# andres2631996/bikg_graph_explainability_public

Hardware: AMD Instinct MI355X
Metric: perturbation-samples/sec (masked GNN fwd) per query node; 1/2/4/8 GPU (higher is better)
Workload: dtype fp32

## Files before the change

bikg_graph_explainability_public_amd/_lib.py:

```python
import ctypes
import os

import torch

_HERE = os.path.dirname(os.path.abspath(__file__))
LIB_PATH = os.path.join(_HERE, "libxpgnn.so")
ABI_VERSION = 27
MAX_TERMS = 8

ACT = {None: 0, "identity": 0, "relu": 1, "sigmoid": 2, "tanh": 3, "leaky_relu": 4, "elu": 5}
TERM = {"gcn": 0, "mean": 1, "root": 2, "att": 3, "sum": 4, "max": 5, "rel": 6}
REL_NORM = {"mean": 0, "sum": 1}
POOL = {None: 0, "mean": 1, "sum": 2, "max": 3}

c_i32, c_i64, c_f32, c_vp = ctypes.c_int32, ctypes.c_int64, ctypes.c_float, ctypes.c_void_p


class NativeLibraryError(RuntimeError):
    pass


class FitExchangeError(RuntimeError):
    """The multi-workgroup surrogate fit's cross-workgroup exchange timed out (its workgroups
    were not all resident on the GPU at once): the fit's outputs are invalid."""
# ... 32 lines not shown


class WlmParams(ctypes.Structure):
    _fields_ = [("lr", c_f32), ("l1_lambda", c_f32), ("beta1", c_f32), ("beta2", c_f32),
                ("eps", c_f32), ("weight_decay", c_f32)]


_SIGS = {
    "xpg_abi_version": ([], c_i32),
    "xpg_last_error": ([], ctypes.c_char_p),
    "xpg_pack_masks": ([c_vp, c_i64, c_i64, c_vp, c_vp], c_i32),
    "xpg_unpack_masks": ([c_vp, c_i64, c_i64, c_vp, c_vp], c_i32),
    "xpg_sample_shapley": ([ctypes.c_uint64, c_i64, c_i64, c_i64, c_vp, c_vp], c_i32),
    "xpg_sample_shapley_counts": ([ctypes.c_uint64, c_i64, c_i64, c_i64, c_vp, c_vp, c_vp], c_i32),
    "xpg_sample_shapley_dev": ([c_vp, c_i64, c_i64, c_i64, c_vp, c_vp], c_i32),
    "xpg_sample_shapley_sets": ([c_vp, c_i32, c_i64, c_i64, c_vp, c_vp], c_i32),
    "xpg_plan_arrays_build": ([c_i64, c_i32, c_vp, c_vp, c_vp, c_vp, c_vp, c_i64, c_i32, c_vp, c_vp], c_i32),
    "xpg_plan_arrays_take": ([c_vp, c_vp], c_i32),
    "xpg_plan_arrays_free": ([c_vp], c_i32),
    "xpg_mt19937_mask_bits": ([c_vp, c_vp, c_vp, c_i64, c_i64, c_vp], c_i32),
    "xpg_mt19937_repeat_draws": ([c_vp, c_vp, c_vp, c_i32, c_i64, ctypes.c_float, ctypes.c_float, c_i32, c_vp,
                                  c_vp], c_i32),
    "xpg_mt19937_community_bits": ([c_vp, c_vp, c_vp, c_i64, c_i32, c_vp, c_vp, c_vp, c_i32, c_i64,
                                    c_vp], c_i32),
    "xpg_sample_communities": ([ctypes.c_uint64, c_i64, c_i64, c_i32, c_vp, c_i32, c_i64, c_i32, c_vp, c_vp,
                                c_vp, c_vp, c_vp], c_i32),
    "xpg_sample_communities_rows": ([ctypes.c_uint64, c_i64, c_i64, c_i64, c_i32, c_vp, c_i32, c_i64, c_i32, c_vp, c_vp,
                                c_vp, c_vp, c_vp], c_i32),
    "xpg_sampler_describe": ([c_i32, c_i64, c_i64, c_i32, c_i32, ctypes.c_char_p, ctypes.c_size_t], c_i32),
    "xpg_edge_keep": ([c_vp, c_i64, c_i64, c_vp, c_vp, c_i64, c_vp, c_vp], c_i32),
    "xpg_rows_no_edge": ([c_vp, c_i64, c_i64, c_vp, c_vp, c_i64, c_vp, c_vp], c_i32),
    "xpg_popcount_rows": ([c_vp, c_i64, c_i64, c_vp, c_vp], c_i32),
    "xpg_shap_kernel": ([c_vp, c_i64, c_i64, c_vp, c_vp], c_i32),
    "xpg_dense": ([c_vp, c_i64, c_i64, c_vp, c_i64, c_i64, c_vp, c_i64, c_i64, ctypes.c_int,
                   c_vp, c_i64, c_vp], c_i32),
    "xpg_forward_workspace": ([ctypes.POINTER(ForwardPlanDesc), c_i64,
                               ctypes.POINTER(ctypes.c_size_t)], c_i32),
    "xpg_masked_forward": ([ctypes.POINTER(ForwardPlanDesc), c_vp, c_i64, c_vp, c_vp,
                            ctypes.c_size_t, c_vp], c_i32),
    "xpg_forward_describe": ([ctypes.POINTER(ForwardPlanDesc), c_i64, ctypes.c_char_p,
                              ctypes.c_size_t], c_i32),
    "xpg_wide_variants": ([ctypes.c_char_p, ctypes.c_size_t], c_i32),
    "xpg_pool_workspace": ([c_i64, c_i64, c_i64, ctypes.POINTER(ctypes.c_size_t)], c_i32),
    "xpg_pool_rows": ([c_vp, c_i64, c_i64, c_i64, c_i32, c_vp, c_vp, ctypes.c_size_t, c_vp], c_i32),
    "xpg_pool_describe": ([c_i64, c_i64, c_i64, c_i32, ctypes.c_char_p, ctypes.c_size_t], c_i32),
    "xpg_profile_enable": ([ctypes.c_int], c_i32),
    "xpg_profile_read": ([c_vp, c_vp, c_i32], c_i32),
    "xpg_wlm_workspace": ([c_i64, c_i64, c_i64, c_i64, ctypes.POINTER(ctypes.c_size_t)], c_i32),
    "xpg_wlm_plan": ([c_i64, c_i64, c_i64, c_i64, ctypes.POINTER(c_i32), ctypes.POINTER(c_i32)], c_i32),
    "xpg_wlm_fit": ([c_i64, c_vp, c_i64, c_i64, c_i64, c_vp, c_vp, ctypes.POINTER(WlmParams), c_i64,
                     c_vp, c_vp, c_vp, c_vp, c_vp, c_vp, c_vp, ctypes.c_size_t, c_vp], c_i32),
    "xpg_wlm_fit_from": ([c_i64, c_vp, c_i64, c_i64, c_i64, c_vp, c_vp, ctypes.POINTER(WlmParams), c_vp,
                          c_vp, c_vp, c_vp, c_vp, c_vp, c_vp, c_vp, ctypes.c_size_t, c_vp], c_i32),
    "xpg_wlm_prepare": ([c_i64, c_vp, c_i64, c_i64, c_i64, c_vp, c_vp, ctypes.POINTER(WlmParams), c_vp,
                         c_vp, c_vp, c_vp, c_vp, ctypes.c_size_t, c_vp], c_i32),
    "xpg_wlm_fit_prepared": ([c_i64, c_vp, c_i64, c_i64, c_i64, c_vp, ctypes.POINTER(WlmParams), c_vp,
                              c_vp, c_vp, c_vp, c_vp, c_vp, c_vp, ctypes.c_size_t, c_vp], c_i32),
    "xpg_wlm_fit_steps": ([c_i64, c_vp, c_i64, c_i64, c_i64, c_vp, ctypes.POINTER(WlmParams), c_vp, c_vp,
                           c_vp, c_vp, ctypes.c_size_t, c_vp], c_i32),
    "xpg_wlm_fit_losses": ([c_i64, c_i64, c_i64, c_i64, c_vp, ctypes.POINTER(WlmParams), c_vp, c_vp, c_vp,
                            c_vp, ctypes.c_size_t, c_vp], c_i32),
    "xpg_khop_workspace": ([c_i64, c_i64, ctypes.POINTER(ctypes.c_size_t)], c_i32),
    "xpg_khop_subgraph": ([c_vp, c_i64, c_i64, c_i64, c_i32, c_vp, c_vp, c_vp, c_vp, c_vp, c_vp,
                           ctypes.c_size_t, c_vp], c_i32),
}

# ... 62 lines not shown
```

bikg_graph_explainability_public_amd/csrc/xpgnn.hip:

```cpp
#include <hip/hip_runtime.h>

#include <algorithm>
#include <cmath>
#include <cstdlib>
#include <cstdint>
#include <cstring>
#include <string>
#include <mutex>
#include <unordered_map>
#include <unordered_set>
#include <vector>

#include "../../include/xpgnn.h"
#include "host_rng.h"
#include "plan_host.h"

namespace {

thread_local std::string g_err;

int fail(int code, const std::string& msg) {
  g_err = msg;
  return code;
}
// ... 456 lines not shown
  if (k < 0.0 || k > n) return 0.0;
  double kx = k;
  if (kx > n / 2 && n > 0) kx = n - kx;
  if (kx >= 0 && kx < 20) {
    double num = 1.0, den = 1.0;
    const int kk = static_cast<int>(kx);
    for (int i = 1; i < 1 + kk; ++i) {
      num *= i + n - kx;
      den *= i;
      if (fabs(num) > 1e50) {
        num /= den;
        den = 1.0;
      }
    }
    return num / den;
  }
  return exp(lgamma(n + 1.0) - lgamma(k + 1.0) - lgamma(n - k + 1.0));
}

__device__ __forceinline__ double clean_inf(double v) { return (isinf(v) || isnan(v)) ? 0.0 : v; }

__device__ double block_sum_d(double v, double* red) {
#pragma unroll
  for (int off = 32; off > 0; off >>= 1) v += __shfl_xor(v, off, 64);
  const int wv = threadIdx.x >> 6, nw = blockDim.x >> 6;
  __syncthreads();
  if ((threadIdx.x & 63) == 0) red[wv] = v;
  __syncthreads();
  double s = 0.0;
  for (int i = 0; i < nw; ++i) s += red[i];
  return s;
}

__global__ void k_shap_exact(const int32_t* __restrict__ cnt, int64_t rows, int64_t cols,
                             double* __restrict__ out) {
  const int64_t r = blockIdx.x * (int64_t)blockDim.x + threadIdx.x;
  if (r >= rows) return;
  const int64_t Mi = cols - 1;
  const double M = static_cast<double>(Mi);
  const int64_t k = cnt[r];
  const double choose = binom_d(M + 1.0, static_cast<double>(k));
  out[r] = clean_inf(M / (choose * static_cast<double>(Mi + 1 - k) * static_cast<double>(k)));
}

__device__ __forceinline__ double shap_approx_row(int64_t k, int64_t Mi, int ref) {
  const double M = static_cast<double>(Mi);
  int64_t idx = static_cast<int64_t>(static_cast<float>(k * 1000) / static_cast<float>(Mi));
  idx = idx < 0 ? 0 : (idx > ref - 1 ? ref - 1 : idx);
  const double choose = (binom_d(static_cast<double>(ref), static_cast<double>(idx)) + 1e-10) * M / 1000.0;
  return M / (choose * static_cast<double>(k) * static_cast<double>(Mi - k));
}

__global__ void k_shap_approx_rows(const int32_t* __restrict__ cnt, int64_t rows, int64_t cols,
                                   double* __restrict__ out) {
  const int64_t r = blockIdx.x * (int64_t)blockDim.x + threadIdx.x;
  if (r < rows) out[r] = shap_approx_row(cnt[r], cols - 1, 1000);
}

__global__ __launch_bounds__(1024) void k_shap_approx_finish(const int32_t* __restrict__ cnt,
                                                             int64_t rows, int64_t cols,
                                                             double* __restrict__ out) {
  const int64_t Mi = cols - 1;
  int ref = 1000;
  for (;;) {
    bool found = false;
    for (int64_t base = 0; base < rows && !found; base += blockDim.x) {
      const int64_t r = base + threadIdx.x;
      found = __syncthreads_or(r < rows && !(out[r] == 0.0)) != 0;
    }
    if (found) break;
    ref = static_cast<int>(0.9 * static_cast<double>(ref));
    if (!(ref > 0)) break;
    __syncthreads();
    for (int64_t r = threadIdx.x; r < rows; r += blockDim.x) out[r] = shap_approx_row(cnt[r], Mi, ref);
    __syncthreads();
  }
}

__global__ void k_shap_clean(int64_t rows, double* __restrict__ out) {
  const int64_t r = blockIdx.x * (int64_t)blockDim.x + threadIdx.x;
  if (r < rows) out[r] = clean_inf(out[r]);
}

__device__ __forceinline__ float half_wave_sum(float x) {
  x += __int_as_float(__builtin_amdgcn_update_dpp(0, __float_as_int(x), 0xB1, 0xF, 0xF, false));
  x += __int_as_float(__builtin_amdgcn_update_dpp(0, __float_as_int(x), 0x4E, 0xF, 0xF, false));
  x += __int_as_float(__builtin_amdgcn_update_dpp(0, __float_as_int(x), 0x124, 0xF, 0xF, false));
  x += __int_as_float(__builtin_amdgcn_update_dpp(0, __float_as_int(x), 0x128, 0xF, 0xF, false));
  const auto r = __builtin_amdgcn_permlane16_swap(__float_as_uint(x), __float_as_uint(x), false, false);
  return __uint_as_float(r[0]) + __uint_as_float(r[1]);
}

template <int NT, bool HEAD = false>
__global__ __launch_bounds__(256) void k_dense(const float* __restrict__ A, int64_t M, int64_t lda,
                                               const float* __restrict__ W, int64_t ldw, int k_pad,
                                               const float* __restrict__ bias, int n_real, int act,
                                               float* __restrict__ C, int64_t ldc,
                                               const int32_t* __restrict__ row_type, int64_t type_mod,
                                               int bias_ld, int n_groups, const float* __restrict__ hw = nullptr,
                                               const float* __restrict__ hb = nullptr, int hact = 0,
                                               float* __restrict__ y = nullptr) {
  const int lane = threadIdx.x & 63;
  const int64_t wv = blockIdx.x * (int64_t)(blockDim.x >> 6) + (threadIdx.x >> 6);
  const int cg = static_cast<int>(wv % n_groups);
  const int64_t m0 = (wv / n_groups) * 32;
  if (m0 >= M) return;
  const int c0 = cg * NT * 32;
  W += (int64_t)c0 * ldw;
  bias += c0;
  C += c0;
  if (HEAD) hw += c0;
  n_real -= c0;
  const int i = lane & 31, h = lane >> 5;
  const int64_t arow = m0 + i;
// ... 1156 lines not shown
    }
  }
}

__device__ __forceinline__ void rows_dense(const float* A, int K, const float* W, int ldw,
                                           const float* __restrict__ bias, int n_real, int n_pad, int act,
                                           float* out, int wave, int lane) {
  for (int o0 = wave * 4; o0 < n_pad; o0 += 4 * kRowsWaves) {
    float acc[4] = {0.f, 0.f, 0.f, 0.f};
#pragma unroll 2
    for (int kc = 0; kc < K; kc += 4) {
      float av[4];
      float4 wv[4];
#pragma unroll
      for (int i = 0; i < 4; ++i) av[i] = A[(kc + i) * 64 + lane];
#pragma unroll
      for (int q = 0; q < 4; ++q) wv[q] = *reinterpret_cast<const float4*>(W + (int64_t)(o0 + q) * ldw + kc);
#pragma unroll
      for (int q = 0; q < 4; ++q) {
        acc[q] = fmaf(av[0], wv[q].x, acc[q]);
        acc[q] = fmaf(av[1], wv[q].y, acc[q]);
        acc[q] = fmaf(av[2], wv[q].z, acc[q]);
        acc[q] = fmaf(av[3], wv[q].w, acc[q]);
      }
    }
#pragma unroll
    for (int q = 0; q < 4; ++q) {
      const int o = o0 + q;
      if (o < n_pad) out[o * 64 + lane] = o < n_real ? act_apply(acc[q] + bias[o], act) : 0.f;
    }
  }
}

template <int FS, bool SUMK>
__device__ __forceinline__ void rows_h1(const RowsFwdArgs& a, const float* lds, int s, int fo, int lane,
                                        float (&h)[FS]) {
  const int* li = reinterpret_cast<const int*>(lds);
#pragma unroll
  for (int f = 0; f < FS; ++f) h[f] = 0.f;
  const int tf0 = li[a.o_l1tgt + s];
  for (int k = 0; k < a.n_terms1; ++k) {
    const int kind = a.kind1[k], r = a.rel1[k];
    const float* T = lds + a.o_tab + k * a.n0 * a.f1_pad + fo;
    const float* dvr = lds + a.o_dv + r * a.n0 * 64 + lane;
    float cself, cedge_t;
    if (kind == XPG_TERM_ROOT) {
      cself = 1.f;
      cedge_t = 0.f;
    } else {
      const float kt = lds[a.o_kt + (r * a.n1 + tf0) * 64 + lane];
      if (kind == XPG_TERM_GCN) {
        const float dt = inv_sqrt_deg(kt);
        cself = dt * dt;
        cedge_t = kt >= 0.f ? dt : 0.f;
      } else {
        const int sm = li[a.o_l1smul + r * a.n1 + s];
        const float cnt = kt + static_cast<float>(sm);
        const float inv = SUMK && kind == XPG_TERM_SUM ? 1.f : 1.f / (cnt > 1.f ? cnt : 1.f);
        cself = kt >= 0.f ? static_cast<float>(sm) * inv : 0.f;
        cedge_t = kt >= 0.f ? inv : 0.f;
      }
    }
    {
      float v[FS];
      ld_fs<FS>(T + tf0 * a.f1_pad, v);
#pragma unroll
      for (int f = 0; f < FS; ++f) h[f] = fmaf(cself, v[f], h[f]);
    }
    if (kind == XPG_TERM_ROOT) continue;
    const int* pp = li + a.o_l1ptr + r * (a.n1 + 1);
    const int e0 = pp[s], e1 = pp[s + 1];
    const float gmul = kind == XPG_TERM_GCN ? cedge_t : 0.f;
    const float mmul = kind == XPG_TERM_GCN ? 0.f : cedge_t;
    constexpr int EB = 4;
    for (int wb = e0; wb < e1; wb += 64) {
      const int ne = min(64, e1 - wb);
      const int vsrc = li[a.o_l1f0 + wb + min(lane, ne - 1)];
      for (int i0 = 0; i0 < ne; i0 += EB) {
        int u[EB];
        float d[EB], v[EB][FS];
#pragma unroll
        for (int q = 0; q < EB; ++q) u[q] = rdl(vsrc, min(i0 + q, ne - 1));
#pragma unroll
        for (int q = 0; q < EB; ++q) d[q] = dvr[u[q] * 64];
#pragma unroll
        for (int q = 0; q < EB; ++q) ld_fs<FS>(T + u[q] * a.f1_pad, v[q]);
#pragma unroll
        for (int q = 0; q < EB; ++q) {
          const float valid = static_cast<float>(i0 + q < ne);
          const float c = valid * fmaf(d[q], gmul, fminf(d[q] * 1e30f, 1.f) * mmul);
#pragma unroll
          for (int f = 0; f < FS; ++f) h[f] = fmaf(c, v[q][f], h[f]);
        }
      }
    }
  }
#pragma unroll
  for (int f = 0; f < FS; ++f) {
    const int fg = fo + f;
    h[f] = fg < a.f1_out ? act_apply(h[f] + a.bias1[fg], a.act1) : 0.f;
  }
}

template <int FS, bool SUMK = false>
__global__ __launch_bounds__(1024) void k_rows_forward(const RowsFwdArgs a) {
  extern __shared__ __attribute__((aligned(16))) float lds[];
  int* li = reinterpret_cast<int*>(lds);
  const int tid = threadIdx.x, lane = tid & 63;
  const int wave = __builtin_amdgcn_readfirstlane(tid >> 6);
  __shared__ int blk_s;
  if (a.ctl) {
    if (tid == 0) {
      const int x = xcc_id();
      const int busy = __hip_atomic_load(g_xcd_busy + x, __ATOMIC_RELAXED, __HIP_MEMORY_SCOPE_AGENT);
      const int cap = a.cus_per_xcd - busy > 1 ? a.cus_per_xcd - busy : 1;
      const int slot = __hip_atomic_fetch_add(a.ctl + 1 + x, 1, __ATOMIC_RELAXED, __HIP_MEMORY_SCOPE_AGENT);
      blk_s = slot < cap ? 0 : -1;
    }
    __syncthreads();
    if (blk_s < 0) return;
  }
#ifdef XPG_WLM_STAMPS
  uint64_t stamp_acc[8] = {0, 0, 0, 0, 0, 0, 0, 0};
  uint64_t stamp_last = __builtin_amdgcn_s_memtime();
#endif
  {
    const int n4 = a.n0 * a.f1_pad / 4;
    for (int k = 0; k < a.n_terms1; ++k) {
// ... 2301 lines not shown
  for (int i = 0; i < kStepDw; ++i) d[i] = __builtin_amdgcn_readlane(v, i);
  WlmStep s;
  s.ybar = __hiloint2double(static_cast<int>(d[1]), static_cast<int>(d[0]));
  s.ksum = __hiloint2double(static_cast<int>(d[3]), static_cast<int>(d[2]));
  s.vy = __hiloint2double(static_cast<int>(d[5]), static_cast<int>(d[4]));
  s.cg = __hiloint2double(static_cast<int>(d[7]), static_cast<int>(d[6]));
  s.step_size = __uint_as_float(d[8]);
  s.bc2_sqrt = __uint_as_float(d[9]);
  s.inv_bc2 = __uint_as_float(d[10]);
  s.pad = 0.f;
  return s;
}

template <int B>
__device__ __forceinline__ float quad_bcast(float x) {
  return __int_as_float(__builtin_amdgcn_mov_dpp(__float_as_int(x), B | (B << 2) | (B << 4) | (B << 6), 0xF, 0xF, false));
}

__device__ __forceinline__ void quad_table_entries(float x, float* dst) {
  const float x0 = quad_bcast<0>(x), x1 = quad_bcast<1>(x), x2 = quad_bcast<2>(x), x3 = quad_bcast<3>(x);
  const int q = threadIdx.x & 3;
#pragma unroll
  for (int i = 0; i < 4; ++i) {
    const int vv = 4 * q + i;
    float s = 0.f;
    s += (vv & 1) ? x0 : 0.f;
    s += (vv & 2) ? x1 : 0.f;
    s += (vv & 4) ? x2 : 0.f;
    s += (vv & 8) ? x3 : 0.f;
    dst[vv] = s;
  }
}

template <int CPL, int STG>
__global__ __launch_bounds__(1024) void k_wlm_fit_mc(
    const uint32_t* __restrict__ bits, const uint32_t* __restrict__ colbits, int64_t rows, int cols, int words,
    int batch, int bw, int P, int wpp, int n_ds, int64_t n_fits, int xcd_local,
    const double* __restrict__ kern,
    const WlmStep* __restrict__ stp, xpg_wlm_params Pm, float* __restrict__ wg, float* __restrict__ mg,
    float* __restrict__ vg, float* __restrict__ p_hist, float* __restrict__ w_hist, uint64_t* xp,
    uint32_t* err, uint32_t spin_limit, int fault_part, uint32_t epoch_host, int plain_ok,
    const uint32_t* __restrict__ ep_dev) {
  uint32_t epoch = (epoch_host + (ep_dev ? *ep_dev : 0u)) & 0xFFFFu;
  if (epoch == 0u) epoch = 1u;
  static_assert(sizeof(WlmStep) == 48, "WlmStep is read as 12 dwords");
  extern __shared__ __attribute__((aligned(16))) char smem[];
  __shared__ int abort_s;
  const int tid = threadIdx.x, lane = tid & 63, wave = tid >> 6;
  if (tid == 0) abort_s = 0;
  int64_t f;
  int part;
  if (xcd_local) {
    const int64_t k = blockIdx.x >> 3, g = k / P;
    part = static_cast<int>(k - g * P);
    f = g * 8 + (blockIdx.x & 7);
    if (f >= n_fits) return;
  } else {
    f = blockIdx.x / P;
    part = static_cast<int>(blockIdx.x - f * P);
  }
  const int my_xcc = xcc_id();
  if (tid == 0) __hip_atomic_fetch_add(g_xcd_busy + my_xcc, 1, __ATOMIC_RELAXED, __HIP_MEMORY_SCOPE_AGENT);
  const int64_t nsteps = (rows + batch - 1) / batch;
  const int w_lo = min(words, part * wpp), w_hi = min(words, w_lo + wpp);
  const int ow = w_hi - w_lo;
  const int c_lo = w_lo * 32, ncol = max(0, min(cols, w_hi * 32) - c_lo);
// ... 103 lines not shown
        __builtin_amdgcn_s_sleep(1);
        gx = ld64_sc1(xc + lane);
        ++n;
      }
      same = static_cast<uint32_t>(gx >> 32) == htag && static_cast<uint32_t>(gx) == xcc;
    }
    const bool all = __ballot(!same) == 0ull && plain_ok;
    if (lane == 0) plain_s = all ? 1 : 0;
  }
  XPG_MC_STORE(0)
  lds_barrier();
  const bool plain = plain_s != 0;
#ifdef XPG_WLM_STAMPS
  uint64_t stamp_acc[8] = {0, 0, 0, 0, 0, 0, 0, 0};
  uint64_t stamp_last = __builtin_amdgcn_s_memtime();
#endif

  for (int64_t t = 0; t < nsteps; ++t) {
    const int64_t r0 = t * batch;
    const int B = static_cast<int>((rows - r0) < batch ? (rows - r0) : batch);
    const WlmStep sc = wlm_step_from_lanes(stw);
    uint64_t* xs = xp + (t & 1) * P * (int64_t)batch;
    const uint32_t tag = (epoch << 16) | static_cast<uint32_t>(t + 1);
    const int j = wave * 64 + lane;
    const bool prow = wave < nrb && j < B;
    float pown = 0.f;
    if (wave < nrb) {
      if (j < B) {
        const uint32_t* row = Rb + j * rp;
        if (ow <= 4) {
          uint32_t wv[4];
#pragma unroll
          for (int h = 0; h < 4; ++h) wv[h] = row[h < ow ? h : 0];
#pragma unroll
          for (int h = 0; h < 4; ++h) {
            const float x = nib8(T + ((h < ow ? h : 0) * 8) * kTabPitch, wv[h]);
            pown += h < ow ? x : 0.f;
          }
        } else {
          for (int kw = 0; kw < ow; kw += 2) {
            uint32_t wv[2];
#pragma unroll
            for (int h = 0; h < 2; ++h) wv[h] = row[kw + h < ow ? kw + h : kw];
#pragma unroll
            for (int h = 0; h < 2; ++h) {
              const float x = nib8(T + ((kw + h < ow ? kw + h : kw) * 8) * kTabPitch, wv[h]);
              pown += kw + h < ow ? x : 0.f;
            }
          }
        }
        const bool skip_pub = fault_part == part && f == 0 && t == 0;
        if (!skip_pub) {
          const uint64_t gv = (static_cast<uint64_t>(tag) << 32) | __float_as_uint(pown);
          if (plain)
            __hip_atomic_store(xs + part * (int64_t)batch + j, gv, __ATOMIC_RELAXED, __HIP_MEMORY_SCOPE_WORKGROUP);
          else
            st64_sc1(xs + part * (int64_t)batch + j, gv);
        }
      }
    }
    XPG_STAMP(0)
    if (t + 1 < nsteps) {
      XPG_MC_LOAD(t + 1)
      stw = lane < kStepDw ? stp32[(t + 1) * kStepDw + lane] : 0u;
    }
#pragma unroll
    for (int c = 0; c < CPL; ++c) {
      const int i = (wave + 16 * c) * cw + col_lo;
      if (sl == 0 && i < ncol) w_hist[t * cols + i] = w[c];
    }
    XPG_STAMP(1)
// ... 2456 lines not shown

int xpg_edge_keep(const uint32_t* bits, int64_t rows, int64_t cols, const int32_t* src, const int32_t* dst,
                  int64_t n_edges, uint8_t* keep, xpg_stream_t stream) {
  XPG_REQ(rows >= 0 && cols > 0 && n_edges >= 0, "edge_keep: bad shape");
  const int64_t n = rows * n_edges;
  if (n == 0) return XPG_OK;
  hipLaunchKernelGGL(k_edge_keep, dim3(static_cast<unsigned>(cdiv(n, 256))), dim3(256), 0, S(stream), bits, rows, words_of(cols), src, dst, n_edges, keep);
  XPG_LAUNCHED();
  return XPG_OK;
}

int xpg_rows_no_edge(const uint32_t* bits, int64_t rows, int64_t cols, const int32_t* src, const int32_t* dst,
                     int64_t n_edges, uint8_t* empty, xpg_stream_t stream) {
  XPG_REQ(rows >= 0 && cols > 0 && n_edges >= 0, "rows_no_edge: bad shape");
  if (rows == 0) return XPG_OK;
  const int rpw = 4;
  hipLaunchKernelGGL(k_rows_no_edge, dim3(static_cast<unsigned>(cdiv(cdiv(rows, rpw), 4))), dim3(256), 0, S(stream),
                     bits, rows, words_of(cols), src, dst, n_edges, empty, rpw);
  XPG_LAUNCHED();
  return XPG_OK;
}

int xpg_popcount_rows(const uint32_t* bits, int64_t rows, int64_t cols, int32_t* counts, xpg_stream_t stream) {
  XPG_REQ(rows >= 0 && cols > 0, "popcount: bad shape");
  if (rows == 0) return XPG_OK;
  hipLaunchKernelGGL(k_popcount, dim3(static_cast<unsigned>(cdiv(rows, 4))), dim3(256), 0, S(stream), bits, rows, words_of(cols), counts);
  XPG_LAUNCHED();
  return XPG_OK;
}

int xpg_shap_kernel(const int32_t* counts, int64_t rows, int64_t cols, double* kernel_out, xpg_stream_t stream) {
  XPG_REQ(rows >= 0 && cols > 1, "shap_kernel: need cols > 1");
  if (rows == 0) return XPG_OK;
  if (cols - 1 <= 1000)
    hipLaunchKernelGGL(k_shap_exact, dim3(static_cast<unsigned>(cdiv(rows, 256))), dim3(256), 0, S(stream), counts,
                       rows, cols, kernel_out);
  else {
    hipLaunchKernelGGL(k_shap_approx_rows, dim3(static_cast<unsigned>(cdiv(rows, 256))), dim3(256), 0, S(stream),
                       counts, rows, cols, kernel_out);
    XPG_LAUNCHED();
    hipLaunchKernelGGL(k_shap_approx_finish, dim3(1), dim3(1024), 0, S(stream), counts, rows, cols, kernel_out);
    XPG_LAUNCHED();
    hipLaunchKernelGGL(k_shap_clean, dim3(static_cast<unsigned>(cdiv(rows, 256))), dim3(256), 0, S(stream), rows,
                       kernel_out);
  }
  XPG_LAUNCHED();
  return XPG_OK;
}

int xpg_dense(const float* A, int64_t M, int64_t lda, const float* W, int64_t ldw, int64_t k_pad, const float* bias,
              int64_t n_real, int64_t n_pad, int act, float* C, int64_t ldc, xpg_stream_t stream) {
  return launch_dense(A, M, lda, W, ldw, k_pad, bias, n_real, n_pad, act, C, ldc, S(stream));
}

int xpg_profile_enable(int on) {
  for (ProfRec& r : g_prof) {
    (void)hipEventDestroy(r.a);
    (void)hipEventDestroy(r.b);
  }
  g_prof.clear();
  g_prof_on = on != 0;
  return XPG_OK;
}

int xpg_profile_read(double* ms, int64_t* launches, int32_t n_slots) {
  XPG_REQ(ms != nullptr && launches != nullptr && n_slots > 0, "profile_read: bad arguments");
  for (int i = 0; i < n_slots; ++i) {
    ms[i] = 0.0;
    launches[i] = 0;
  }
  int rc = XPG_OK;
  for (ProfRec& r : g_prof) {
    float t = 0.f;
    if (hipEventSynchronize(r.b) != hipSuccess || hipEventElapsedTime(&t, r.a, r.b) != hipSuccess) rc = XPG_EHIP;
    if (r.slot >= 0 && r.slot < n_slots) {
      ms[r.slot] += t;
      ++launches[r.slot];
    }
// ... 800 lines not shown
```

bikg_graph_explainability_public_amd/engine.py:

```python
import contextlib
import ctypes
import gc
import itertools
import math

import numpy as np
import torch

from . import _lib
from ._lib import ACT, REL_NORM, TERM, ForwardPlanDesc, HeadDesc, LayerDesc, WlmParams, call, ptr
from .program import fold_attention, relation_weights, stack_attention


def _rup(x, m):
    return ((int(x) + m - 1) // m) * m


def words_of(cols):
    return (int(cols) + 31) // 32


def pack_masks(mask: torch.Tensor) -> torch.Tensor:
    _lib.require_device(mask, "mask")
    m = mask.contiguous()
# ... 283 lines not shown
def rows_no_edge(bits, cols, src, dst):
    _lib.require_device(bits, "bits")
    rows = bits.shape[0]
    s = src.to(device=bits.device, dtype=torch.int32).contiguous()
    d = dst.to(device=bits.device, dtype=torch.int32).contiguous()
    out = torch.empty(rows, dtype=torch.uint8, device=bits.device)
    call("xpg_rows_no_edge", ptr(bits), rows, cols, ptr(s), ptr(d), s.numel(), ptr(out),
         _lib.stream_of(bits.device))
    return out.view(torch.bool)


def khop_subgraph(node_idx: int, num_hops: int, edge_index: torch.Tensor, num_nodes: int):
    _lib.require_device(edge_index, "edge_index")
    dev = edge_index.device
    ei = edge_index.to(torch.int64).contiguous()
    E, N, seed = ei.shape[1], int(num_nodes), int(node_idx)
    if not 0 <= seed < N:
        raise IndexError(f"k_hop_subgraph: node {seed} out of range for {N} nodes")
    nbytes = ctypes.c_size_t(0)
    call("xpg_khop_workspace", N, E, ctypes.byref(nbytes))
    ws = _workspace(dev, nbytes.value)
    subset = torch.empty(N, dtype=torch.int64, device=dev)
    sub = torch.empty((2, max(E, 1)), dtype=torch.int64, device=dev)
    emask = torch.empty(E, dtype=torch.uint8, device=dev)
    counts = torch.empty(4, dtype=torch.int64, device=dev)
    call("xpg_khop_subgraph", ptr(ei), E, N, seed, int(num_hops), ptr(subset), ptr(sub),
         ptr(sub[1]), ptr(emask), ptr(counts), ptr(ws), ws.numel(), _lib.stream_of(dev))
    n_sub, n_e, inv, bad = counts.tolist()
    if bad:
        raise IndexError("k_hop_subgraph: edge_index holds node ids outside [0, num_nodes)")
    return subset[:n_sub], sub[:, :n_e].contiguous(), counts[2:3], emask.view(torch.bool)


def shap_kernel(bits: torch.Tensor, cols: int, counts: torch.Tensor = None,
                out: torch.Tensor = None, scratch: torch.Tensor = None) -> torch.Tensor:
    _lib.require_device(bits, "bits")
    rows = bits.shape[0]
    if out is None:
        out = torch.empty(rows, dtype=torch.float64, device=bits.device)
    elif out.dtype != torch.float64 or out.numel() != rows or not out.is_contiguous():
        raise ValueError("out must be a contiguous float64 [rows] tensor")
    st = _lib.stream_of(bits.device)
    if counts is None:
        if scratch is None:
            scratch = torch.empty(rows, dtype=torch.int32, device=bits.device)
        elif scratch.dtype != torch.int32 or scratch.numel() != rows or not scratch.is_contiguous():
            raise ValueError("scratch must be a contiguous int32 [rows] tensor")
        counts = scratch
        call("xpg_popcount_rows", ptr(bits), rows, cols, ptr(counts), st)
    else:
        _lib.require_device(counts, "counts")
        if counts.dtype != torch.int32 or counts.numel() != rows:
            raise ValueError("counts must be int32 [rows]")
        counts = counts.contiguous()
    call("xpg_shap_kernel", ptr(counts), rows, cols, ptr(out), st)
    return out


def dense(A: torch.Tensor, W: torch.Tensor, bias, act=None, n_real=None) -> torch.Tensor:
    dev = A.device
    M, K = A.shape
    N = W.shape[0] if n_real is None else n_real
    k_pad, n_pad = _rup(K, 8), _rup(max(N, 1), 32)
    Ap = A if (K == k_pad and A.is_contiguous()) else \
        torch.nn.functional.pad(A.float(), (0, k_pad - K)).contiguous()
    Wp = torch.zeros((n_pad, k_pad), dtype=torch.float32, device=dev)
    Wp[:W.shape[0], :K] = W
    bp = torch.zeros(n_pad, dtype=torch.float32, device=dev)
    if bias is not None:
        bp[:bias.shape[0]] = bias
    C = torch.empty((M, n_pad), dtype=torch.float32, device=dev)
    call("xpg_dense", ptr(Ap), M, k_pad, ptr(Wp), k_pad, k_pad, ptr(bp), N, n_pad,
         ACT[act], ptr(C), n_pad, _lib.stream_of(dev))
    return C[:, :N]


PROF_SLOTS = ("wide_bits", "wide_f0", "wide_degree", "wide_l1", "wide_l2")


def profile_enable(on=True):
    _lib.check(_lib.load().xpg_profile_enable(1 if on else 0))


def profile_read():
    n = len(PROF_SLOTS)
    ms = (ctypes.c_double * n)()
    cnt = (ctypes.c_int64 * n)()
# ... 746 lines not shown
```

include/xpgnn.h:

```cpp
#ifndef XPGNN_H
#define XPGNN_H

#include <stddef.h>
#include <stdint.h>

#ifdef __cplusplus
extern "C" {
#endif

#define XPG_ABI_VERSION 27
#define XPG_MAX_TERMS 8

typedef void* xpg_stream_t;

enum xpg_status { XPG_OK = 0, XPG_EINVAL = 1, XPG_EHIP = 2, XPG_ENOSPC = 3 };

enum xpg_act { XPG_ACT_NONE = 0, XPG_ACT_RELU = 1, XPG_ACT_SIGMOID = 2, XPG_ACT_TANH = 3,
               XPG_ACT_LEAKY_RELU = 4, XPG_ACT_ELU = 5 };

enum xpg_term { XPG_TERM_GCN = 0,
                XPG_TERM_MEAN = 1,
                XPG_TERM_ROOT = 2,
                XPG_TERM_ATT = 3,
                XPG_TERM_SUM = 4,
// ... 23 lines not shown
                               int32_t n_comm, const int32_t* comm_ptr, const int32_t* comm_cols,
                               const int32_t* blocks, int32_t n_blocks, int64_t rows, uint32_t* bits);
int xpg_plan_arrays_build(int64_t S, int32_t n_rel, const int64_t* rel_ptr, const int64_t* src,
                          const int64_t* dst, const int64_t* eid, const int64_t* queries, int64_t nq,
                          int32_t L, void** handle, int64_t* sizes);
int xpg_plan_arrays_take(void* handle, int64_t* out);
int xpg_plan_arrays_free(void* handle);
int xpg_sample_shapley_counts(uint64_t seed, int64_t row_offset, int64_t rows, int64_t cols,
                              uint32_t* bits, int32_t* counts, xpg_stream_t stream);
int xpg_sample_communities(uint64_t seed, int64_t rows, int64_t cols, int32_t n_comm,
                           const int32_t* blocks, int32_t n_blocks, int64_t src_rows,
                           int32_t shuffle, const int32_t* col_ptr, const int32_t* col_comm,
                           uint32_t* bits, int32_t* prow, xpg_stream_t stream);
int xpg_sample_communities_rows(uint64_t seed, int64_t row_offset, int64_t rows, int64_t cols,
                                int32_t n_comm, const int32_t* blocks, int32_t n_blocks,
                                int64_t src_rows, int32_t shuffle, const int32_t* col_ptr,
                                const int32_t* col_comm, uint32_t* bits, int32_t* prow,
                                xpg_stream_t stream);

enum xpg_sampler { XPG_SAMPLER_SHAPLEY = 0, XPG_SAMPLER_COMMUNITIES = 1 };
int xpg_sampler_describe(int32_t kind, int64_t rows, int64_t cols, int32_t n_comm, int32_t n_blocks,
                         char* buf, size_t n);

int xpg_edge_keep(const uint32_t* bits, int64_t rows, int64_t cols, const int32_t* src,
                  const int32_t* dst, int64_t n_edges, uint8_t* keep, xpg_stream_t stream);

int xpg_rows_no_edge(const uint32_t* bits, int64_t rows, int64_t cols, const int32_t* src,
                     const int32_t* dst, int64_t n_edges, uint8_t* empty, xpg_stream_t stream);

int xpg_popcount_rows(const uint32_t* bits, int64_t rows, int64_t cols, int32_t* counts,
                      xpg_stream_t stream);
int xpg_shap_kernel(const int32_t* counts, int64_t rows, int64_t cols, double* kernel_out,
                    xpg_stream_t stream);

int xpg_dense(const float* A, int64_t M, int64_t lda, const float* W, int64_t ldw,
              int64_t k_pad, const float* bias, int64_t n_real, int64_t n_pad, int act,
              float* C, int64_t ldc, xpg_stream_t stream);

typedef struct xpg_term_desc {
  int32_t kind;
  int32_t rel;
  const float* table;
  int32_t dst_type;
  int32_t heads, head_ch;
  float neg_slope;
  int32_t self_loops;
  const float* att_src;
  const float* att_dst;
  int32_t n_slices;
  int32_t norm;
  const float* coef;
} xpg_term_desc;

typedef struct xpg_layer_desc {
  int32_t n_terms;
  int32_t act;
  int32_t f_in_pad;
  int32_t f_out;
  int32_t f_out_pad;
  int32_t n_tgt;
  int32_t n_edges;
  const int32_t* tgt_prev;
  const int32_t* tgt_f0;
  const int32_t* agg_ptr;
  const int32_t* agg_src;
  const int32_t* agg_f0;
// ... 103 lines not shown
```

Measured before the change: 145.2 million.

## Fuse popcount into SHAP kernel weights and specialize layer-1 edge gather

```diff
diff --git a/bikg_graph_explainability_public_amd/_lib.py b/bikg_graph_explainability_public_amd/_lib.py
--- a/bikg_graph_explainability_public_amd/_lib.py
+++ b/bikg_graph_explainability_public_amd/_lib.py
@@ -88,6 +88,7 @@
     "xpg_rows_no_edge": ([c_vp, c_i64, c_i64, c_vp, c_vp, c_i64, c_vp, c_vp], c_i32),
     "xpg_popcount_rows": ([c_vp, c_i64, c_i64, c_vp, c_vp], c_i32),
     "xpg_shap_kernel": ([c_vp, c_i64, c_i64, c_vp, c_vp], c_i32),
+    "xpg_shap_kernel_bits": ([c_vp, c_i64, c_i64, c_vp, c_vp, c_vp], c_i32),
     "xpg_dense": ([c_vp, c_i64, c_i64, c_vp, c_i64, c_i64, c_vp, c_i64, c_i64, ctypes.c_int,
                    c_vp, c_i64, c_vp], c_i32),
     "xpg_forward_workspace": ([ctypes.POINTER(ForwardPlanDesc), c_i64,
diff --git a/bikg_graph_explainability_public_amd/csrc/xpgnn.hip b/bikg_graph_explainability_public_amd/csrc/xpgnn.hip
--- a/bikg_graph_explainability_public_amd/csrc/xpgnn.hip
+++ b/bikg_graph_explainability_public_amd/csrc/xpgnn.hip
@@ -560,6 +560,73 @@
 __global__ void k_shap_clean(int64_t rows, double* __restrict__ out) {
   const int64_t r = blockIdx.x * (int64_t)blockDim.x + threadIdx.x;
   if (r < rows) out[r] = clean_inf(out[r]);
+}
+
+constexpr int kShapRows = 64;
+
+__device__ int popc_row_serial(const uint32_t* __restrict__ row, int words) {
+  int c = 0;
+  for (int w = 0; w < words; ++w) c += __popc(row[w]);
+  return c;
+}
+
+__global__ __launch_bounds__(256) void k_shap_bits(const uint32_t* __restrict__ bits, int64_t rows, int words,
+                                                   int64_t cols, int lg, int32_t* __restrict__ counts,
+                                                   double* __restrict__ out) {
+  __shared__ int cnt_s[kShapRows];
+  const int tid = threadIdx.x;
+  const int64_t row0 = blockIdx.x * (int64_t)kShapRows;
+  const int G = 1 << lg, g = tid & (G - 1);
+  for (int rl = tid >> lg; rl < kShapRows; rl += 256 >> lg) {
+    const int64_t r = row0 + rl;
+    int c = 0;
+    if (r < rows) {
+      const uint32_t* row = bits + r * words;
+      int c1 = 0, c2 = 0, c3 = 0, w = g;
+      for (; w + 3 * G < words; w += 4 * G) {
+        c += __popc(row[w]);
+        c1 += __popc(row[w + G]);
+        c2 += __popc(row[w + 2 * G]);
+        c3 += __popc(row[w + 3 * G]);
+      }
+      for (; w < words; w += G) c += __popc(row[w]);
+      c += c1 + c2 + c3;
+    }
+    for (int off = G >> 1; off > 0; off >>= 1) c += __shfl_xor(c, off, 64);
+    if (g == 0) cnt_s[rl] = c;
+  }
+  __syncthreads();
+  const int64_t r = row0 + tid;
+  const bool mine = tid < kShapRows && r < rows;
+  const int64_t Mi = cols - 1;
+  const int64_t k = mine ? cnt_s[tid] : 0;
+  if (mine && counts) counts[r] = static_cast<int32_t>(k);
+  if (Mi <= 1000) {
+    if (mine) {
+      const double M = static_cast<double>(Mi);
+      const double choose = binom_d(M + 1.0, static_cast<double>(k));
+      out[r] = clean_inf(M / (choose * static_cast<double>(Mi + 1 - k) * static_cast<double>(k)));
+    }
+    return;
+  }
+  double v = mine ? shap_approx_row(k, Mi, 1000) : 0.0;
+  if (!__syncthreads_or(mine && !(v == 0.0))) {
+    int ref = 1000;
+    for (;;) {
+      bool found = false;
+      for (int64_t base = 0; base < rows && !found; base += blockDim.x) {
+        const int64_t q = base + tid;
+        const bool nz = q < rows && !(shap_approx_row(popc_row_serial(bits + q * words, words), Mi, ref) == 0.0);
+        found = __syncthreads_or(nz) != 0;
+      }
+      if (found) break;
+      const int next = static_cast<int>(0.9 * static_cast<double>(ref));
+      if (!(next > 0)) break;
+      ref = next;
+    }
+    if (mine) v = shap_approx_row(k, Mi, ref);
+  }
+  if (mine) out[r] = clean_inf(v);
 }
 
 __device__ __forceinline__ float half_wave_sum(float x) {
@@ -1782,6 +1849,36 @@
   }
 }
 
+template <int FS, bool GCNK>
+__device__ __forceinline__ void rows_h1_edges(const int* l1f0, const float* T, const float* dvr, int f1_pad, int e0,
+                                              int e1, int lane, float ce, float (&h)[FS]) {
+  constexpr int EB = 4;
+  auto batch = [&](int vsrc, int i0, auto nb) {
+    constexpr int N = decltype(nb)::value;
+    int u[N];
+    float d[N], v[N][FS];
+#pragma unroll
+    for (int q = 0; q < N; ++q) u[q] = rdl(vsrc, i0 + q);
+#pragma unroll
+    for (int q = 0; q < N; ++q) d[q] = dvr[u[q] * 64];
+#pragma unroll
+    for (int q = 0; q < N; ++q) ld_fs<FS>(T + u[q] * f1_pad, v[q]);
+#pragma unroll
+    for (int q = 0; q < N; ++q) {
+      const float c = GCNK ? d[q] * ce : (d[q] > 0.f ? ce : 0.f);
+#pragma unroll
+      for (int f = 0; f < FS; ++f) h[f] = fmaf(c, v[q][f], h[f]);
+    }
+  };
+  for (int wb = e0; wb < e1; wb += 64) {
+    const int ne = min(64, e1 - wb);
+    const int vsrc = l1f0[wb + min(lane, ne - 1)];
+    int i0 = 0;
+    for (; i0 + EB <= ne; i0 += EB) batch(vsrc, i0, std::integral_constant<int, EB>());
+    for (; i0 < ne; ++i0) batch(vsrc, i0, std::integral_constant<int, 1>());
+  }
+}
+
 template <int FS, bool SUMK>
 __device__ __forceinline__ void rows_h1(const RowsFwdArgs& a, const float* lds, int s, int fo, int lane,
                                         float (&h)[FS]) {
@@ -1820,30 +1917,8 @@
     if (kind == XPG_TERM_ROOT) continue;
     const int* pp = li + a.o_l1ptr + r * (a.n1 + 1);
     const int e0 = pp[s], e1 = pp[s + 1];
-    const float gmul = kind == XPG_TERM_GCN ? cedge_t : 0.f;
-    const float mmul = kind == XPG_TERM_GCN ? 0.f : cedge_t;
-    constexpr int EB = 4;
-    for (int wb = e0; wb < e1; wb += 64) {
-      const int ne = min(64, e1 - wb);
-      const int vsrc = li[a.o_l1f0 + wb + min(lane, ne - 1)];
-      for (int i0 = 0; i0 < ne; i0 += EB) {
-        int u[EB];
-        float d[EB], v[EB][FS];
-#pragma unroll
-        for (int q = 0; q < EB; ++q) u[q] = rdl(vsrc, min(i0 + q, ne - 1));
-#pragma unroll
-        for (int q = 0; q < EB; ++q) d[q] = dvr[u[q] * 64];
-#pragma unroll
-        for (int q = 0; q < EB; ++q) ld_fs<FS>(T + u[q] * a.f1_pad, v[q]);
-#pragma unroll
-        for (int q = 0; q < EB; ++q) {
-          const float valid = static_cast<float>(i0 + q < ne);
-          const float c = valid * fmaf(d[q], gmul, fminf(d[q] * 1e30f, 1.f) * mmul);
-#pragma unroll
-          for (int f = 0; f < FS; ++f) h[f] = fmaf(c, v[q][f], h[f]);
-        }
-      }
-    }
+    if (kind == XPG_TERM_GCN) rows_h1_edges<FS, true>(li + a.o_l1f0, T, dvr, a.f1_pad, e0, e1, lane, cedge_t, h);
+    else rows_h1_edges<FS, false>(li + a.o_l1f0, T, dvr, a.f1_pad, e0, e1, lane, cedge_t, h);
   }
 #pragma unroll
   for (int f = 0; f < FS; ++f) {
@@ -6919,6 +6994,19 @@
     hipLaunchKernelGGL(k_shap_clean, dim3(static_cast<unsigned>(cdiv(rows, 256))), dim3(256), 0, S(stream), rows,
                        kernel_out);
   }
+  XPG_LAUNCHED();
+  return XPG_OK;
+}
+
+int xpg_shap_kernel_bits(const uint32_t* bits, int64_t rows, int64_t cols, int32_t* counts_out, double* kernel_out,
+                         xpg_stream_t stream) {
+  XPG_REQ(rows >= 0 && cols > 1, "shap_kernel_bits: need cols > 1");
+  if (rows == 0) return XPG_OK;
+  const int words = words_of(cols);
+  int lg = 0;
+  while (lg < 6 && (8 << lg) < words) ++lg;
+  hipLaunchKernelGGL(k_shap_bits, dim3(static_cast<unsigned>(cdiv(rows, kShapRows))), dim3(256), 0, S(stream), bits,
+                     rows, words, cols, lg, counts_out, kernel_out);
   XPG_LAUNCHED();
   return XPG_OK;
 }
diff --git a/bikg_graph_explainability_public_amd/engine.py b/bikg_graph_explainability_public_amd/engine.py
--- a/bikg_graph_explainability_public_amd/engine.py
+++ b/bikg_graph_explainability_public_amd/engine.py
@@ -339,6 +339,13 @@
     return subset[:n_sub], sub[:, :n_e].contiguous(), counts[2:3], emask.view(torch.bool)
 
 
+def popcount_rows(bits: torch.Tensor, cols: int) -> torch.Tensor:
+    _lib.require_device(bits, "bits")
+    counts = torch.empty(bits.shape[0], dtype=torch.int32, device=bits.device)
+    call("xpg_popcount_rows", ptr(bits), bits.shape[0], cols, ptr(counts), _lib.stream_of(bits.device))
+    return counts
+
+
 def shap_kernel(bits: torch.Tensor, cols: int, counts: torch.Tensor = None,
                 out: torch.Tensor = None, scratch: torch.Tensor = None) -> torch.Tensor:
     _lib.require_device(bits, "bits")
@@ -349,17 +356,15 @@
         raise ValueError("out must be a contiguous float64 [rows] tensor")
     st = _lib.stream_of(bits.device)
     if counts is None:
-        if scratch is None:
-            scratch = torch.empty(rows, dtype=torch.int32, device=bits.device)
-        elif scratch.dtype != torch.int32 or scratch.numel() != rows or not scratch.is_contiguous():
+        if scratch is not None and (scratch.dtype != torch.int32 or scratch.numel() != rows
+                                    or not scratch.is_contiguous()):
             raise ValueError("scratch must be a contiguous int32 [rows] tensor")
-        counts = scratch
-        call("xpg_popcount_rows", ptr(bits), rows, cols, ptr(counts), st)
-    else:
-        _lib.require_device(counts, "counts")
-        if counts.dtype != torch.int32 or counts.numel() != rows:
-            raise ValueError("counts must be int32 [rows]")
-        counts = counts.contiguous()
+        call("xpg_shap_kernel_bits", ptr(bits), rows, cols, ptr(scratch), ptr(out), st)
+        return out
+    _lib.require_device(counts, "counts")
+    if counts.dtype != torch.int32 or counts.numel() != rows:
+        raise ValueError("counts must be int32 [rows]")
+    counts = counts.contiguous()
     call("xpg_shap_kernel", ptr(counts), rows, cols, ptr(out), st)
     return out
 
diff --git a/include/xpgnn.h b/include/xpgnn.h
--- a/include/xpgnn.h
+++ b/include/xpgnn.h
@@ -79,6 +79,8 @@
                       xpg_stream_t stream);
 int xpg_shap_kernel(const int32_t* counts, int64_t rows, int64_t cols, double* kernel_out,
                     xpg_stream_t stream);
+int xpg_shap_kernel_bits(const uint32_t* bits, int64_t rows, int64_t cols, int32_t* counts_out,
+                         double* kernel_out, xpg_stream_t stream);
 
 int xpg_dense(const float* A, int64_t M, int64_t lda, const float* W, int64_t ldw,
               int64_t k_pad, const float* bias, int64_t n_real, int64_t n_pad, int act,
```

Result: no change. 145.1 million (-0.1%).

## Fuse row popcount and Shapley kernel weights into one kernel

Applied to the files above, without the earlier changes.

```diff
diff --git a/bikg_graph_explainability_public_amd/_lib.py b/bikg_graph_explainability_public_amd/_lib.py
--- a/bikg_graph_explainability_public_amd/_lib.py
+++ b/bikg_graph_explainability_public_amd/_lib.py
@@ -88,6 +88,7 @@
     "xpg_rows_no_edge": ([c_vp, c_i64, c_i64, c_vp, c_vp, c_i64, c_vp, c_vp], c_i32),
     "xpg_popcount_rows": ([c_vp, c_i64, c_i64, c_vp, c_vp], c_i32),
     "xpg_shap_kernel": ([c_vp, c_i64, c_i64, c_vp, c_vp], c_i32),
+    "xpg_shap_from_bits": ([c_vp, c_i64, c_i64, c_vp, c_vp, c_vp], c_i32),
     "xpg_dense": ([c_vp, c_i64, c_i64, c_vp, c_i64, c_i64, c_vp, c_i64, c_i64, ctypes.c_int,
                    c_vp, c_i64, c_vp], c_i32),
     "xpg_forward_workspace": ([ctypes.POINTER(ForwardPlanDesc), c_i64,
diff --git a/bikg_graph_explainability_public_amd/csrc/xpgnn.hip b/bikg_graph_explainability_public_amd/csrc/xpgnn.hip
--- a/bikg_graph_explainability_public_amd/csrc/xpgnn.hip
+++ b/bikg_graph_explainability_public_amd/csrc/xpgnn.hip
@@ -512,15 +512,10 @@
   return s;
 }
 
-__global__ void k_shap_exact(const int32_t* __restrict__ cnt, int64_t rows, int64_t cols,
-                             double* __restrict__ out) {
-  const int64_t r = blockIdx.x * (int64_t)blockDim.x + threadIdx.x;
-  if (r >= rows) return;
-  const int64_t Mi = cols - 1;
+__device__ __forceinline__ double shap_exact_row(int64_t k, int64_t Mi) {
   const double M = static_cast<double>(Mi);
-  const int64_t k = cnt[r];
   const double choose = binom_d(M + 1.0, static_cast<double>(k));
-  out[r] = clean_inf(M / (choose * static_cast<double>(Mi + 1 - k) * static_cast<double>(k)));
+  return M / (choose * static_cast<double>(Mi + 1 - k) * static_cast<double>(k));
 }
 
 __device__ __forceinline__ double shap_approx_row(int64_t k, int64_t Mi, int ref) {
@@ -531,35 +526,98 @@
   return M / (choose * static_cast<double>(k) * static_cast<double>(Mi - k));
 }
 
-__global__ void k_shap_approx_rows(const int32_t* __restrict__ cnt, int64_t rows, int64_t cols,
-                                   double* __restrict__ out) {
-  const int64_t r = blockIdx.x * (int64_t)blockDim.x + threadIdx.x;
-  if (r < rows) out[r] = shap_approx_row(cnt[r], cols - 1, 1000);
-}
-
-__global__ __launch_bounds__(1024) void k_shap_approx_finish(const int32_t* __restrict__ cnt,
-                                                             int64_t rows, int64_t cols,
-                                                             double* __restrict__ out) {
+constexpr int kShapRows = 64;
+constexpr int kShapThreads = 256;
+
+template <bool BITS>
+__device__ void shap_block_counts(const uint32_t* __restrict__ bits, int words,
+                                  const int32_t* __restrict__ counts, int64_t base, int n, int* cnt_s) {
+  const int tid = threadIdx.x;
+  __syncthreads();
+  if (!BITS) {
+    if (tid < n) cnt_s[tid] = counts[base + tid];
+    __syncthreads();
+    return;
+  }
+  if (tid < kShapRows) cnt_s[tid] = 0;
+  __syncthreads();
+  const uint32_t* p = bits + base * words;
+  const int64_t total = static_cast<int64_t>(n) * words;
+  const int dq = kShapThreads / words, dr = kShapThreads - dq * words;
+  int row = tid / words, rem = tid - row * words;
+  int cur = row, acc = 0;
+  for (int64_t i = tid; i < total; i += 8 * kShapThreads) {
+    uint32_t v[8];
+#pragma unroll
+    for (int u = 0; u < 8; ++u) {
+      const int64_t e = i + u * kShapThreads;
+      v[u] = e < total ? p[e] : 0u;
+    }
+#pragma unroll
+    for (int u = 0; u < 8; ++u) {
+      if (row != cur) {
+        if (acc) atomicAdd(cnt_s + cur, acc);
+        cur = row;
+        acc = 0;
+      }
+      acc += __popc(v[u]);
+      rem += dr;
+      row += dq;
+      if (rem >= words) {
+        rem -= words;
+        ++row;
+      }
+    }
+  }
+  if (acc) atomicAdd(cnt_s + cur, acc);
+  __syncthreads();
+}
+
+template <bool BITS>
+__device__ bool shap_any_nonzero(const uint32_t* __restrict__ bits, int words, const int32_t* __restrict__ counts,
+                                 int64_t rows, int64_t Mi, int ref, int* cnt_s) {
+  for (int64_t base = 0; base < rows; base += kShapRows) {
+    const int n = static_cast<int>(rows - base < kShapRows ? rows - base : kShapRows);
+    shap_block_counts<BITS>(bits, words, counts, base, n, cnt_s);
+    const bool live = static_cast<int>(threadIdx.x) < n;
+    const double v = live ? shap_approx_row(cnt_s[threadIdx.x], Mi, ref) : 0.0;
+    if (__syncthreads_or(live && !(v == 0.0))) return true;
+  }
+  return false;
+}
+
+template <bool BITS>
+__global__ __launch_bounds__(kShapThreads) void k_shap_one(const uint32_t* __restrict__ bits, int words,
+                                                           const int32_t* __restrict__ counts_in,
+                                                           int32_t* __restrict__ counts_out, int64_t rows,
+                                                           int64_t cols, double* __restrict__ out) {
+  __shared__ int cnt_s[kShapRows];
+  const int tid = threadIdx.x;
+  const int64_t base = blockIdx.x * static_cast<int64_t>(kShapRows);
+  const int n = static_cast<int>(rows - base < kShapRows ? rows - base : kShapRows);
   const int64_t Mi = cols - 1;
+  shap_block_counts<BITS>(bits, words, counts_in, base, n, cnt_s);
+  const bool mine = tid < n;
+  const int64_t k = mine ? cnt_s[tid] : 0;
+  if (BITS && mine) counts_out[base + tid] = static_cast<int32_t>(k);
+  if (Mi <= 1000) {
+    if (mine) out[base + tid] = clean_inf(shap_exact_row(k, Mi));
+    return;
+  }
+  const double v = mine ? shap_approx_row(k, Mi, 1000) : 0.0;
+  if (__syncthreads_or(mine && !(v == 0.0))) {
+    if (mine) out[base + tid] = clean_inf(v);
+    return;
+  }
   int ref = 1000;
-  for (;;) {
-    bool found = false;
-    for (int64_t base = 0; base < rows && !found; base += blockDim.x) {
-      const int64_t r = base + threadIdx.x;
-      found = __syncthreads_or(r < rows && !(out[r] == 0.0)) != 0;
-    }
-    if (found) break;
-    ref = static_cast<int>(0.9 * static_cast<double>(ref));
-    if (!(ref > 0)) break;
-    __syncthreads();
-    for (int64_t r = threadIdx.x; r < rows; r += blockDim.x) out[r] = shap_approx_row(cnt[r], Mi, ref);
-    __syncthreads();
-  }
-}
-
-__global__ void k_shap_clean(int64_t rows, double* __restrict__ out) {
-  const int64_t r = blockIdx.x * (int64_t)blockDim.x + threadIdx.x;
-  if (r < rows) out[r] = clean_inf(out[r]);
+  bool found = shap_any_nonzero<BITS>(bits, words, counts_in, rows, Mi, ref, cnt_s);
+  while (!found) {
+    const int nref = static_cast<int>(0.9 * static_cast<double>(ref));
+    if (!(nref > 0)) break;
+    ref = nref;
+    found = shap_any_nonzero<BITS>(bits, words, counts_in, rows, Mi, ref, cnt_s);
+  }
+  if (mine) out[base + tid] = clean_inf(shap_approx_row(k, Mi, ref));
 }
 
 __device__ __forceinline__ float half_wave_sum(float x) {
@@ -4211,6 +4269,14 @@
   }
 }
 
+template <int N>
+__device__ __forceinline__ float nib8_words(const float* T, const uint32_t* wv) {
+  float p = 0.f;
+#pragma unroll
+  for (int h = 0; h < N; ++h) p += nib8(T + (h * 8) * kTabPitch, wv[h]);
+  return p;
+}
+
 template <int CPL, int STG>
 __global__ __launch_bounds__(1024) void k_wlm_fit_mc(
     const uint32_t* __restrict__ bits, const uint32_t* __restrict__ colbits, int64_t rows, int cols, int words,
@@ -4380,11 +4446,8 @@
           uint32_t wv[4];
 #pragma unroll
           for (int h = 0; h < 4; ++h) wv[h] = row[h < ow ? h : 0];
-#pragma unroll
-          for (int h = 0; h < 4; ++h) {
-            const float x = nib8(T + ((h < ow ? h : 0) * 8) * kTabPitch, wv[h]);
-            pown += h < ow ? x : 0.f;
-          }
+          pown = ow == 3 ? nib8_words<3>(T, wv) : ow == 4 ? nib8_words<4>(T, wv)
+                 : ow == 2 ? nib8_words<2>(T, wv) : nib8_words<1>(T, wv);
         } else {
           for (int kw = 0; kw < ow; kw += 2) {
             uint32_t wv[2];
@@ -6907,18 +6970,19 @@
 int xpg_shap_kernel(const int32_t* counts, int64_t rows, int64_t cols, double* kernel_out, xpg_stream_t stream) {
   XPG_REQ(rows >= 0 && cols > 1, "shap_kernel: need cols > 1");
   if (rows == 0) return XPG_OK;
-  if (cols - 1 <= 1000)
-    hipLaunchKernelGGL(k_shap_exact, dim3(static_cast<unsigned>(cdiv(rows, 256))), dim3(256), 0, S(stream), counts,
-                       rows, cols, kernel_out);
-  else {
-    hipLaunchKernelGGL(k_shap_approx_rows, dim3(static_cast<unsigned>(cdiv(rows, 256))), dim3(256), 0, S(stream),
-                       counts, rows, cols, kernel_out);
-    XPG_LAUNCHED();
-    hipLaunchKernelGGL(k_shap_approx_finish, dim3(1), dim3(1024), 0, S(stream), counts, rows, cols, kernel_out);
-    XPG_LAUNCHED();
-    hipLaunchKernelGGL(k_shap_clean, dim3(static_cast<unsigned>(cdiv(rows, 256))), dim3(256), 0, S(stream), rows,
-                       kernel_out);
-  }
+  hipLaunchKernelGGL(k_shap_one<false>, dim3(static_cast<unsigned>(cdiv(rows, kShapRows))), dim3(kShapThreads), 0,
+                     S(stream), nullptr, 0, counts, nullptr, rows, cols, kernel_out);
+  XPG_LAUNCHED();
+  return XPG_OK;
+}
+
+int xpg_shap_from_bits(const uint32_t* bits, int64_t rows, int64_t cols, int32_t* counts_out, double* kernel_out,
+                       xpg_stream_t stream) {
+  XPG_REQ(rows >= 0 && cols > 1, "shap_from_bits: need cols > 1");
+  XPG_REQ(cols <= (int64_t{1} << 30), "shap_from_bits: row too long");
+  if (rows == 0) return XPG_OK;
+  hipLaunchKernelGGL(k_shap_one<true>, dim3(static_cast<unsigned>(cdiv(rows, kShapRows))), dim3(kShapThreads), 0,
+                     S(stream), bits, words_of(cols), nullptr, counts_out, rows, cols, kernel_out);
   XPG_LAUNCHED();
   return XPG_OK;
 }
diff --git a/bikg_graph_explainability_public_amd/engine.py b/bikg_graph_explainability_public_amd/engine.py
--- a/bikg_graph_explainability_public_amd/engine.py
+++ b/bikg_graph_explainability_public_amd/engine.py
@@ -353,13 +353,12 @@
             scratch = torch.empty(rows, dtype=torch.int32, device=bits.device)
         elif scratch.dtype != torch.int32 or scratch.numel() != rows or not scratch.is_contiguous():
             raise ValueError("scratch must be a contiguous int32 [rows] tensor")
-        counts = scratch
-        call("xpg_popcount_rows", ptr(bits), rows, cols, ptr(counts), st)
-    else:
-        _lib.require_device(counts, "counts")
-        if counts.dtype != torch.int32 or counts.numel() != rows:
-            raise ValueError("counts must be int32 [rows]")
-        counts = counts.contiguous()
+        call("xpg_shap_from_bits", ptr(bits), rows, cols, ptr(scratch), ptr(out), st)
+        return out
+    _lib.require_device(counts, "counts")
+    if counts.dtype != torch.int32 or counts.numel() != rows:
+        raise ValueError("counts must be int32 [rows]")
+    counts = counts.contiguous()
     call("xpg_shap_kernel", ptr(counts), rows, cols, ptr(out), st)
     return out
 
diff --git a/include/xpgnn.h b/include/xpgnn.h
--- a/include/xpgnn.h
+++ b/include/xpgnn.h
@@ -79,6 +79,8 @@
                       xpg_stream_t stream);
 int xpg_shap_kernel(const int32_t* counts, int64_t rows, int64_t cols, double* kernel_out,
                     xpg_stream_t stream);
+int xpg_shap_from_bits(const uint32_t* bits, int64_t rows, int64_t cols, int32_t* counts_out,
+                       double* kernel_out, xpg_stream_t stream);
 
 int xpg_dense(const float* A, int64_t M, int64_t lda, const float* W, int64_t ldw,
               int64_t k_pad, const float* bias, int64_t n_real, int64_t n_pad, int act,
```

Result: no change. 145.1 million before, 143.7 million after (-1.0%).
